# isaac-chandler/cuda-raytracer

Measured on AMD Instinct MI355X. Metric: Mrays/s (live ray segments/s, teapot), higher is better.
Workload: dtype f32

## Files before the change

### cuda-raytracer_amd/csrc/rt_render.hip

```cpp
#include "rt_common.h"

#include <algorithm>
#include <chrono>
#include <cstdio>
#include <cstdlib>
#include <cstring>
#include <string>
#include <thread>
#include <vector>

#include <rccl/rccl.h>

#pragma clang fp contract(off)

int rtamd_render_multi(const rt_scene *scene, const rt_opts *opts, float *fb_out, rt_stats *stats);

using namespace rtamd;

namespace {

#ifndef RT_INFLIGHT
#define RT_INFLIGHT 20
#endif
#ifndef RT_TRACE_OCC
// ... 26 lines not shown
inline int tile_stride(int64_t n_max) {
    return (int)std::max<int64_t>(kTileTarget, (n_max + kSortTile - 1) / kSortTile);
}
constexpr int kBuckets = 65;
constexpr int kInflight = RT_INFLIGHT;
constexpr int kStaggerUs = 4000;
constexpr int kStaggerGroup = 4;
constexpr int kStaggerMinPasses = 8;
constexpr int kStaggerShortUs = 2000;
constexpr int kTraceOccPct = RT_TRACE_OCC;
constexpr uint32_t kDead = 64;
constexpr uint32_t kAccFlag = 0x80000000u;
constexpr int kSpanSlots = 8;
constexpr int kSpanWords = 2 * kSpanSlots;
#ifdef RT_PROFILE
__device__ unsigned long long g_prof[2][14];
#define PROF(i, v) (prof[i] += (v))
#else
#define PROF(i, v) ((void)0)
#endif

struct FastDiv {
    uint32_t m = 0;
    int l = 0;
    static FastDiv of(uint32_t d) {
        FastDiv f;
        if (d > 1) {
            f.l = 32 - __builtin_clz(d - 1);
            f.m = (uint32_t)((((uint64_t)1 << (31 + f.l)) + d - 1) / d);
        }
        return f;
    }
    __device__ __forceinline__ uint32_t div(uint32_t n) const { return l == 0 ? n : (__umulhi(n, m) >> (l - 1)); }
};

struct SlotMap {
    FastDiv by_stripe;
    uint32_t skip, base;
    static SlotMap identity() { return SlotMap{FastDiv::of(0x7fffffffu), 0u, 0u}; }
    static SlotMap of(uint32_t stripe, int count, int index) {
        return SlotMap{FastDiv::of(stripe), (uint32_t)(count - 1) * stripe, (uint32_t)index * stripe};
    }
    __device__ __forceinline__ uint32_t ray(uint32_t s) const { return s + by_stripe.div(s) * skip + base; }
};

template <int FIRST>
__device__ __forceinline__ uint32_t first_ray(const SlotMap &m, uint32_t slot) {
    return FIRST == 2 ? m.ray(slot) : slot;
}

struct PassArgs {
    int rtc;
    uint32_t gen_seed_term;
    FastDiv by_rtc, by_width;
    SlotMap map;
};

__device__ __forceinline__ V3 primary_dir(const DevScene &S, int i, const PassArgs &pa) {
    Rng rng = pcg_seed((uint32_t)i * 0x85810BEAu + pa.gen_seed_term);
    uint32_t z;
    asm volatile("v_mov_b32 %0, 0" : "=v"(z));
    rng.inc += z;
    const uint32_t pixel = pa.by_rtc.div((uint32_t)i);
    const uint32_t yy = pa.by_width.div(pixel);
    const int x = (int)(pixel - yy * (uint32_t)S.width), y = (int)yy;
    const float xc = (x + random01(rng)) * S.inv_w;
    const float yc = (y + random01(rng)) * S.inv_h;
    return normalise(S.tl + xc * S.sr - yc * S.su);
}

#ifndef RT_FUSED_MAX_TRIS
#define RT_FUSED_MAX_TRIS 4096
#endif
#ifndef RT_SORT_GRID
#define RT_SORT_GRID 0
#endif

template <bool SORTED, bool COUNT, int FIRST, bool VSLOT = false>
__global__ __launch_bounds__(kBlock) RT_TRACE_ATTR void trace_kernel(DevScene S, PassArgs pa, const float4 *__restrict__ geo,
                                                       const uint32_t *__restrict__ live_count,
                                                       uint32_t *__restrict__ queue, float2 *__restrict__ hits,
                                                       uint32_t *__restrict__ overflow, Counters *__restrict__ ctr,
                                                       unsigned long long *__restrict__ tspan,
                                                       const uint8_t *__restrict__ slot_bkt = nullptr) {
    __shared__ uint2 stack[(kStackLds + 1) * kBlock];
    const unsigned long long t_start = wall_clock64();
    uint2 *col = stack + threadIdx.x;
    const uint32_t lanes = gridDim.x * kBlock, gl = blockIdx.x * kBlock + threadIdx.x;
    const uint32_t dist_half = lanes * (kStackMax - kStackLds);
    const uint32_t L = __builtin_amdgcn_readfirstlane(*live_count);
    const uint32_t waves = gridDim.x * (kBlock / 64);
    const uint32_t chunk = min((uint32_t)kChunkMax, max((uint32_t)kChunkMin, (L / (4 * waves) + 63) & ~63u));
    uint32_t shard = blockIdx.x % kQueues, tried = 0;
    uint32_t q_next = 0, q_end = 0;
    bool exhausted = false;
    int slot = -1;
    V3 o{0, 0, 0}, d{0, 0, 0};
    float ix = 0, iy = 0, iz = 0, closest = 0;
    bool finite_inv = true;
    bool wave_nonfinite = false;
    int index = -1, sp = 0;
    uint32_t ref = 0;
    int ti = 0, te = 0;
    unsigned pn = 0, iv = 0, tt = 0, nlive = 0;
#ifdef RT_PROFILE
    unsigned long long prof[14] = {0, 0, 0, 0, 0, 0, 0, 0, 0, 0, 0, 0, 0, 0};
#endif
    auto node_step = [&](float4 a, float4 b, float4 c, uint2 kids) -> bool {
        if (COUNT) iv++;
        float t0, t1;
        bool h0, h1;
        slab_pair(a, b, c, o, ix, iy, iz, closest, h0, h1, t0, t1);
        if (__builtin_expect(wave_nonfinite, 0)) {
            float u0, u1;
            const bool g0 = slab(a.x, a.z, b.x, b.z, c.x, c.z, o, ix, iy, iz, closest, u0);
            const bool g1 = slab(a.y, a.w, b.y, b.w, c.y, c.w, o, ix, iy, iz, closest, u1);
            if (!finite_inv) { h0 = g0; h1 = g1; t0 = u0; t1 = u1; }
        }
        const bool both = h0 && h1, any = h0 || h1;
        const bool sel1 = h1 && (!h0 || t0 < t1);
        const uint32_t next_ref = sel1 ? kids.y : kids.x, near_ref = sel1 ? kids.x : kids.y;
        const float next_t = sel1 ? t1 : t0, near_t = sel1 ? t0 : t1;
        col[min(sp, kStackLds) * kBlock] = make_uint2(near_ref, __float_as_uint(near_t));
        if (__builtin_expect(both && sp >= kStackLds, 0)) {
            overflow[(sp - kStackLds) * lanes + gl] = near_ref;
            overflow[dist_half + (sp - kStackLds) * lanes + gl] = __float_as_uint(near_t);
        }
        if (both) sp++;
        ref = any ? next_ref : ref;
        const bool descend = any && !(next_t >= closest);
        bool need = !descend;
        if (descend) {
            if (COUNT) pn++;
            if (ref & kLeaf) {
                leaf_range(S, ref, ti, te);
                need = ti == te;
            }
        }
        return need;
    };
    auto pop_loop = [&](bool need) {
        while (need) {
            PROF(10, 1);
            const bool empty = sp == 0;
            sp = empty ? 0 : sp - 1;
            uint2 e = col[min(sp, kStackLds) * kBlock];
            asm volatile("" : "+v"(e.x), "+v"(e.y));
            if (__builtin_expect(__ballot(sp >= kStackLds) != 0, 0)) {
                if (sp >= kStackLds) {
                    e.x = overflow[(sp - kStackLds) * lanes + gl];
                    e.y = overflow[dist_half + (sp - kStackLds) * lanes + gl];
                }
            }
            const bool take = !empty && !(__uint_as_float(e.y) >= closest);
            slot = empty ? -2 - slot : slot;
            ref = take ? e.x : ref;
            if (COUNT) pn += take ? 1u : 0u;
            const bool leaf = take && (ref & kLeaf);
            if (__builtin_expect(leaf && (ref & kBigLeaf), 0)) {
                leaf_range(S, ref, ti, te);
            } else {
                ti = leaf ? (int)(ref & 0xFFFFFFu) : ti;
                te = leaf ? ti + (int)((ref >> 24) & 0x3Fu) : te;
            }
            need = !empty && (!take || (leaf && ti == te));
        }
    };
    const bool root_internal = !(S.root_ref & kLeaf);
    float4 ra{0, 0, 0, 0}, rb{0, 0, 0, 0}, rc{0, 0, 0, 0};
    uint2 rk{0, 0};
    if (root_internal) {
        const float4 *rr = S.nodes + (size_t)S.root_ref * 4;
        const float4 x0 = rr[0], x1 = rr[1], x2 = rr[2];
        const uint2 k = *reinterpret_cast<const uint2 *>(rr + 3);
#define RT_U(v) __int_as_float(__builtin_amdgcn_readfirstlane(__float_as_int(v)))
        ra = make_float4(RT_U(x0.x), RT_U(x0.y), RT_U(x0.z), RT_U(x0.w));
        rb = make_float4(RT_U(x1.x), RT_U(x1.y), RT_U(x1.z), RT_U(x1.w));
        rc = make_float4(RT_U(x2.x), RT_U(x2.y), RT_U(x2.z), RT_U(x2.w));
#undef RT_U
        rk = make_uint2(__builtin_amdgcn_readfirstlane(k.x), __builtin_amdgcn_readfirstlane(k.y));
    }
    while (true) {
        unsigned long long idle = __ballot(slot < 0);
        if (!exhausted && __popcll(idle) >= (FIRST ? kRefillFirst : kRefill)) {
            PROF(6, 1);
            if (slot <= -2) {
                hits[-2 - slot] = make_float2(closest, __int_as_float(index));
                slot = -1;
            }
            bool fresh = false;
            do {
                bool got = false;
                while (idle && !exhausted) {
                    if (q_next >= q_end) {
                        const uint32_t seg_lo = (uint32_t)(((uint64_t)L * shard) / kQueues);
                        const uint32_t seg_hi = (uint32_t)(((uint64_t)L * (shard + 1)) / kQueues);
                        uint32_t c = 0;
                        if (lane_id() == 0) c = atomicAdd(queue + shard * kQueueStride, chunk);
                        c = __builtin_amdgcn_readfirstlane(__shfl(c, 0)) + seg_lo;
                        if (c >= seg_hi) {
                            shard = (shard + 1) % kQueues;
                            if (++tried == kQueues) exhausted = true;
                            continue;
                        }
                        q_next = c;
                        q_end = min(c + chunk, seg_hi);
                    }
                    const uint32_t avail = q_end - q_next;
                    const uint32_t r = rank_below(idle);
                    const bool take = slot < 0 && r < avail;
                    const unsigned long long took = __ballot(take);
                    if (take) { slot = (int)(q_next + r); fresh = true; got = true; }
                    q_next += (uint32_t)__popcll(took);
                    idle &= ~took;
                }
                if (VSLOT) {
                    if (got && slot_bkt[slot] == kDead) { slot = -1; fresh = false; }
                    idle = __ballot(slot < 0);
                }
            } while (VSLOT && idle && !exhausted);
            if (fresh) {
                {
                    nlive++;
                    if (FIRST) {
                        o = S.cam;
                        d = primary_dir(S, (int)first_ray<FIRST>(pa.map, (uint32_t)slot), pa);
                    } else if (VSLOT) {
                        const float2 *rp = reinterpret_cast<const float2 *>(geo) + (size_t)slot * 3;
                        const float2 r0 = rp[0], r1 = rp[1], r2 = rp[2];
                        o = v3(r0.x, r0.y, r1.x);
                        d = v3(r1.y, r2.x, r2.y);
                    } else {
                        const float4 *rp = geo + (size_t)slot * 2;
                        const float4 r0 = rp[0];
                        const float2 r1 = *reinterpret_cast<const float2 *>(rp + 1);
                        o = v3(r0.x, r0.y, r0.z);
                        d = v3(r0.w, r1.x, r1.y);
                    }
                    ix = 1 / d.x; iy = 1 / d.y; iz = 1 / d.z;
                    finite_inv = __builtin_isfinite(ix) && __builtin_isfinite(iy) && __builtin_isfinite(iz);

                    closest = 1e30f;
                    index = -1;
                    for (int i = 0; i < S.sphere_count; i++) {
                        const float4 sph = S.spheres[i];
                        float t;
                        if (ray_sphere(o, d, v3(sph.x, sph.y, sph.z), sph.w, closest, t)) { closest = t; index = i; }
                    }
                    ref = S.root_ref;
                    sp = 0;
                    if (COUNT) pn++;
                    ti = te = 0;
                    if (ref & kLeaf) {
                        leaf_range(S, ref, ti, te);
                        if (ti == te) {
                            hits[slot] = make_float2(closest, __int_as_float(index));
                            slot = -1;
                        }
                    }
                }
            }
            wave_nonfinite = __ballot(slot >= 0 && !finite_inv) != 0;
            if (root_internal && __ballot(fresh && slot >= 0)) {
                bool need = false;
                if (fresh && slot >= 0) need = node_step(ra, rb, rc, rk);
                pop_loop(need);
            }
        }
        if (!__ballot(slot >= 0)) {
            if (exhausted) break;
            PROF(7, 1);
            continue;
        }
#ifdef RT_PROFILE
        {
            const unsigned long long act = __ballot(slot >= 0), lf = __ballot(slot >= 0 && ti < te);
            PROF(0, 1); PROF(1, __popcll(act)); PROF(2, __popcll(lf));
            PROF(3, lf != 0); PROF(4, (act & ~lf) != 0);
            const bool mixed = lf != 0 && (act & ~lf) != 0;
            PROF(8, mixed);
            if (mixed) PROF(9, min(__popcll(lf), __popcll(act & ~lf)));
            const uintptr_t ra = slot >= 0 ? (uintptr_t)(ti < te ? S.tris + (size_t)ti * 3 : S.nodes + (size_t)ref * 4) : 0;
            const int first = __builtin_ctzll(act);
            const uintptr_t r0 = ((uintptr_t)__shfl((unsigned)(ra >> 32), first) << 32) | __shfl((unsigned)ra, first);
            const unsigned long long same = __ballot(slot >= 0 && ra == r0);
            PROF(12, same == act);
            PROF(13, 4 * __popcll(same) >= 3 * __popcll(act));
        }
#endif
        if (slot < 0) continue;
        bool need = false;
        const bool in_leaf = ti < te;
        const float4 *rec = in_leaf ? S.tris + (size_t)ti * 3 : S.nodes + (size_t)ref * 4;
        const float4 a = rec[0], b = rec[1], c = rec[2];
        uint2 kids = make_uint2(0, 0);
        if (!in_leaf) kids = *reinterpret_cast<const uint2 *>(rec + 3);
        if (in_leaf) {
            const float4 q0 = a, q1 = b;
            const float q2 = c.x;
            if (COUNT) tt++;
            float t;
            const bool hit =
                ray_triangle_flat(o, d, v3(q0.x, q0.y, q0.z), v3(q0.w, q1.x, q1.y), v3(q1.z, q1.w, q2), closest, t);
            closest = hit ? t : closest;
            index = hit ? S.sphere_count + ti : index;
            need = ++ti == te;
        } else {
            need = node_step(a, b, c, kids);
        }
#ifdef RT_PROFILE
        if (__ballot(need)) PROF(5, 1);
#endif
        pop_loop(need);
    }
    if (slot <= -2) hits[-2 - slot] = make_float2(closest, __int_as_float(index));
    Counters *cs = ctr + ((blockIdx.x * (kBlock / 64) + (threadIdx.x >> 6)) & (kCtrSlots - 1));
    const unsigned long long nl = wave_sum(nlive);
    if (COUNT) {
        const unsigned long long a = wave_sum(pn), b = wave_sum(iv), t = wave_sum(tt);
        if (lane_id() == 0) {
            atomicAdd(&cs->pn, a);
            atomicAdd(&cs->iv, b);
            atomicAdd(&cs->tt, t);
            atomicAdd(&cs->st, nl * (unsigned long long)S.sphere_count);
        }
    }
    if (lane_id() == 0 && nl) atomicAdd(&cs->live, nl);
    if (tspan) {
        __syncthreads();
        if (threadIdx.x == 0) {
            atomicMin(&tspan[blockIdx.x % kSpanSlots], t_start);
            atomicMax(&tspan[kSpanSlots + blockIdx.x % kSpanSlots], (unsigned long long)wall_clock64());
        }
    }
#ifdef RT_PROFILE
    prof[11] = wave_sum((unsigned)prof[10]);
    if (lane_id() == 0)
        for (int i = 0; i < 14; i++)
            if (i != 10) atomicAdd(&g_prof[FIRST ? 0 : 1][i], prof[i]);
#endif
}

struct Shaded {
    V3 no, nd, T;
    V3 C;
    uint32_t ray;
    int kind;
    bool acc_holds;
    uint32_t mat;
    bool spec;
};
constexpr uint32_t kSpecBit = 0x80;
struct ShadeIn {
    float2 h;
    uint32_t ray, seed;
    bool acc_holds;
    float4 r0, r1;
    float tz;
};
template <bool SORTED, int FIRST, bool INLINE>
__device__ __forceinline__ ShadeIn shade_in(const PassArgs &pa, int slot, const float4 *__restrict__ geo,
                                            const float *__restrict__ tz, const uint32_t *__restrict__ rid,
                                            const float2 *__restrict__ hits, const uint32_t *__restrict__ seed_of) {
    ShadeIn in{};
    const uint32_t ray0 = first_ray<FIRST>(pa.map, (uint32_t)slot);
    const uint32_t rv = FIRST ? (FIRST == 2 ? ray0 : (uint32_t)slot) : rid[slot];
    in.ray = rv & ~kAccFlag;
    in.acc_holds = (rv & kAccFlag) != 0;
    in.seed = (!FIRST && seed_of) ? seed_of[slot] : (SORTED || FIRST) ? (FIRST == 2 ? ray0 : (uint32_t)slot) : in.ray;
    if (!INLINE) in.h = hits[slot];
    if (!FIRST) {
        in.r0 = geo[(size_t)slot * 2];
        in.r1 = geo[(size_t)slot * 2 + 1];
        in.tz = tz[slot];
    }
    return in;
}
template <bool SORTED, int FIRST, bool INLINE = false, bool SLIM = false>
__device__ __forceinline__ Shaded shade_from(const DevScene &S, const PassArgs &pa, int slot, const ShadeIn &in,
                                             uint32_t seed_term) {
    static_assert(!SLIM || FIRST == 1, "the slim hand-over leaves bounce 0, where T enters as (1,1,1)");
    uint32_t mat = 0;
    bool spec = false;
    Rng rng = pcg_seed(in.seed * 4137874753u + seed_term);
    float closest = in.h.x;
    int index = __float_as_int(in.h.y);
    const uint32_t ray_id = in.ray;
    V3 o, d, T;
    V3 C = v3(0, 0, 0);
    if (FIRST) {
        o = S.cam;
        d = primary_dir(S, (int)(FIRST == 2 ? in.ray : (uint32_t)slot), pa);
        float tx = 1.f, ty = 1.f, tz = 1.f;
        asm volatile("" : "+v"(tx), "+v"(ty), "+v"(tz));
        T = v3(tx, ty, tz);
    } else {
        o = v3(in.r0.x, in.r0.y, in.r0.z);
        d = v3(in.r0.w, in.r1.x, in.r1.y);
        T = v3(in.r1.z, in.r1.w, in.tz);
    }
    if (INLINE) {
        closest = 1e30f;
        index = -1;
        for (int i = 0; i < S.sphere_count; i++) {
            const float4 sph = S.spheres[i];
            float t;
            if (ray_sphere(o, d, v3(sph.x, sph.y, sph.z), sph.w, closest, t)) { closest = t; index = i; }
        }
    }
    V3 no = o, nd = d;
    if (index == -1) {
        C = C + sky_color(S.env, S.env_w, S.env_h, d) * T;
        T = v3(0, 0, 0);
    } else {
        const bool sphere = index < S.sphere_count;
        const uint32_t mi = S.mat_idx[index];
        float4 q = *(sphere ? S.spheres + index : S.tris + (size_t)(index - S.sphere_count) * 3 + 2);
        asm volatile("" : "+v"(q.x), "+v"(q.y), "+v"(q.z), "+v"(q.w));
        no = o + closest * d;
        const V3 normal = sphere ? (1 / q.w) * (no - v3(q.x, q.y, q.z)) : v3(q.y, q.z, q.w);
        const float4 *mp = S.mats + (size_t)mi * 3;
        float4 m0 = mp[0], m1 = mp[1], m2 = mp[2];
        asm volatile("" : "+v"(m0.x), "+v"(m0.y), "+v"(m0.z), "+v"(m0.w), "+v"(m1.x), "+v"(m1.y), "+v"(m1.z),
                          "+v"(m1.w), "+v"(m2.x), "+v"(m2.y), "+v"(m2.z), "+v"(m2.w));
        const Mat m{v3(m0.x, m0.y, m0.z), m0.w, v3(m1.x, m1.y, m1.z), m1.w, v3(m2.x, m2.y, m2.z), m2.w};
        const bool took_spec = scatter(d, normal, m, rng, T, C, nd);
        if (SLIM) {
            spec = took_spec;
            mat = mi;
        }
    }
    return Shaded{no, nd, T, C, ray_id, index == -1 ? 0 : (index < S.sphere_count ? 2 : 1), in.acc_holds, mat, spec};
}
template <bool SORTED, int FIRST, bool INLINE = false, bool SLIM = false>
__device__ __forceinline__ Shaded shade_one(const DevScene &S, const PassArgs &pa, int slot,
                                            const float4 *__restrict__ geo, const float *__restrict__ tz,
                                            const uint32_t *__restrict__ rid, const float2 *__restrict__ hits,
                                            uint32_t seed_term, const uint32_t *__restrict__ seed_of = nullptr) {
    return shade_from<SORTED, FIRST, INLINE, SLIM>(S, pa, slot,
                                                   shade_in<SORTED, FIRST, INLINE>(pa, slot, geo, tz, rid, hits, seed_of),
                                                   seed_term);
}
__device__ __forceinline__ bool has_radiance(V3 c) {
    return ((__float_as_uint(c.x) | __float_as_uint(c.y) | __float_as_uint(c.z)) & 0x7fffffffu) != 0;
}

__device__ __forceinline__ unsigned long long match_bucket(uint32_t b, bool valid);

#ifndef RT_SHADE_WPE
#define RT_SHADE_WPE 8
#endif
#ifndef RT_REPLAY_WPE
#define RT_REPLAY_WPE 8
#endif
#if RT_REPLAY_WPE > 0
#define RT_REPLAY_ATTR __attribute__((amdgpu_waves_per_eu(RT_REPLAY_WPE, RT_REPLAY_WPE)))
#else
#define RT_REPLAY_ATTR
#endif
#if RT_SHADE_WPE > 0
#define RT_SHADE_ATTR __attribute__((amdgpu_waves_per_eu(RT_SHADE_WPE, RT_SHADE_WPE)))
#else
#define RT_SHADE_ATTR
#endif
template <bool SORTED, bool COUNT, int FIRST, bool FUSED, bool INLINE, bool SLIM = false>
__global__ __launch_bounds__(kBlock) RT_SHADE_ATTR void shade_kernel(DevScene S, PassArgs pa, float4 *__restrict__ geo,
                                                       float *__restrict__ tz, uint32_t *__restrict__ rid,
                                                       float4 *__restrict__ acc, uint8_t *__restrict__ bkt,
                                                       const uint32_t *__restrict__ live_count,
                                                       const float2 *__restrict__ hits, uint32_t seed_term, int last,
                                                       Counters *__restrict__ ctr,
                                                       const uint32_t *__restrict__ seed_of = nullptr,
                                                       uint32_t *__restrict__ counts = nullptr, int tiles = 0,
                                                       int home = 0) {
    const int L = (int)__builtin_amdgcn_readfirstlane(*live_count);
    unsigned hit = 0, miss = 0, hit_sphere = 0;
    auto shade_slot = [&](int slot) -> uint32_t {
        const Shaded sh = shade_one<SORTED, FIRST, INLINE, SLIM>(S, pa, slot, geo, tz, rid, hits, seed_term, seed_of);
        const V3 no = sh.no, nd = sh.nd, T = sh.T;
        miss += sh.kind == 0;
        hit += sh.kind != 0;
        hit_sphere += sh.kind == 2;
        const bool dead = is_black(T);
        if (SLIM && !dead && !last) {
            float2 *rec = reinterpret_cast<float2 *>(geo) + (size_t)slot * 3;
            rec[0] = make_float2(no.x, no.y);
            rec[1] = make_float2(no.z, nd.x);
            rec[2] = make_float2(nd.y, nd.z);
            reinterpret_cast<uint16_t *>(tz)[slot] = (uint16_t)sh.mat;
        }
        if (!SLIM && !FUSED && !dead && !last) {
            geo[(size_t)slot * 2] = make_float4(no.x, no.y, no.z, nd.x);
            geo[(size_t)slot * 2 + 1] = make_float4(nd.y, nd.z, T.x, T.y);
            tz[slot] = T.z;
        }
        const bool term = has_radiance(sh.C);
        if (dead || last || (term && !(FIRST && home))) {
            V3 C = sh.C;
            const uint32_t dst = sh.ray;
            if (sh.acc_holds) {
                const float4 a = acc[dst];
                C = v3(a.y, a.z, a.w) + sh.C;
            }
            typedef float f4v __attribute__((ext_vector_type(4)));
            if (dead || last)
                __builtin_nontemporal_store(f4v{T.z, C.x, C.y, C.z}, reinterpret_cast<f4v *>(acc + dst));
            else
                acc[dst] = make_float4(T.z, C.x, C.y, C.z);
        }
        if (!SLIM && !FUSED && !dead && !last && (FIRST || (term && !sh.acc_holds)))
            rid[slot] = sh.ray | (term || sh.acc_holds ? kAccFlag : 0u);
        const uint32_t bk = dead ? kDead : (SORTED ? bucket_of(no, nd, S.min_coord, S.inv_dim) : 0u);
        if (!last) bkt[slot] = (uint8_t)(bk | (SLIM && !dead && sh.spec ? kSpecBit : 0u));
        return bk;
    };
    if (counts && !last) {
        __shared__ uint32_t h[kBuckets];
        const int R = tile_rounds(L), span = kBlock * R;
        for (int tile = blockIdx.x; tile * span < L; tile += gridDim.x) {
            for (int b = threadIdx.x; b < kBuckets; b += kBlock) h[b] = 0;
            __syncthreads();
            const int base = tile * span;
            const int rounds = min(R, (L - base + kBlock - 1) / kBlock);
            for (int r = 0; r < rounds; r++) {
                const int slot = base + r * kBlock + threadIdx.x;
                const bool valid = slot < L;
                const uint32_t bk = valid ? shade_slot(slot) : 0u;
                const unsigned long long peers = match_bucket(bk, valid);
                if (valid && rank_below(peers) == 0) atomicAdd(&h[bk], (uint32_t)__popcll(peers));
            }
            __syncthreads();
            for (int b = threadIdx.x; b < kBuckets; b += kBlock) counts[(size_t)b * tiles + tile] = h[b];
            __syncthreads();
        }
    } else {
        for (int base = blockIdx.x * kBlock; base < L; base += gridDim.x * kBlock) {
            const int slot = base + threadIdx.x;
            if (slot < L) (void)shade_slot(slot);
        }
    }
    if (INLINE) {
        Counters *cs = ctr + ((blockIdx.x * (kBlock / 64) + (threadIdx.x >> 6)) & (kCtrSlots - 1));
        const unsigned long long nl = wave_sum(hit + miss);
        if (lane_id() == 0 && nl) {
            atomicAdd(&cs->live, nl);
            if (COUNT) {
                atomicAdd(&cs->pn, nl);
                atomicAdd(&cs->st, nl * (unsigned long long)S.sphere_count);
            }
        }
    }
    if (COUNT) {
        Counters *cs = ctr + ((blockIdx.x * (kBlock / 64) + (threadIdx.x >> 6)) & (kCtrSlots - 1));
        const unsigned long long h = wave_sum(hit), m = wave_sum(miss), hs = wave_sum(hit_sphere);
        if (lane_id() == 0 && (h | m)) {
            atomicAdd(&cs->hits, h);
            atomicAdd(&cs->misses, m);
            atomicAdd(&cs->hits_sphere, hs);
        }
    }
}

__global__ void fill_live_kernel(uint32_t *__restrict__ live, uint32_t n, int count, uint32_t *__restrict__ queue,
                                 unsigned long long *__restrict__ tspan) {
    const int i = blockIdx.x * blockDim.x + threadIdx.x;
    if (i < count) live[i] = n;
    for (int k = i; k < count * kQueues * kQueueStride; k += blockDim.x) queue[k] = 0;
    if (tspan)
        for (int k = i; k < kSpanWords * count; k += blockDim.x) tspan[k] = (k % kSpanWords) >= kSpanSlots ? 0ull : ~0ull;
}

// ... 269 lines not shown
    if (threadIdx.x == 0) *dst = src ? *src : v;
}

template <bool SORTED, int FIRST, bool INLINE>
__global__ __launch_bounds__(kBlock) RT_REPLAY_ATTR void sort_scatter_shade_kernel(DevScene S, PassArgs pa,
                                                                    const uint8_t *__restrict__ bkt_in,
                                                                    const float4 *__restrict__ geo_in,
                                                                    const float *__restrict__ tz_in,
                                                                    const uint32_t *__restrict__ rid_in,
                                                                    const float2 *__restrict__ hits, uint32_t seed_term,
                                                                    const uint32_t *__restrict__ live_count, int tiles,
                                                                    const uint32_t *__restrict__ offsets,
                                                                    const uint32_t *__restrict__ totals,
                                                                    float4 *__restrict__ geo_out,
                                                                    float *__restrict__ tz_out,
                                                                    uint32_t *__restrict__ rid_out,
                                                                    float4 *__restrict__ acc = nullptr,
                                                                    uint32_t *__restrict__ home_of = nullptr,
                                                                    uint32_t home_base = 0) {
    const bool homes = FIRST == 1 && home_of != nullptr;
    const int n = (int)*live_count;
    __shared__ uint32_t run[kBuckets];
    __shared__ uint32_t wcount[kBlock / 64][kBuckets];
    const int R = tile_rounds(n), span = kBlock * R;
    for (int tile = blockIdx.x; tile * span < n; tile += gridDim.x) {
        bucket_runs(run, offsets, totals, tiles, tile);
        for (int k = threadIdx.x; k < (kBlock / 64) * kBuckets; k += kBlock) (&wcount[0][0])[k] = 0;
        __syncthreads();
        const int wave = threadIdx.x >> 6;
        const int base = tile * span;
        const int rounds = min(R, (n - base + kBlock - 1) / kBlock);
        for (int r = 0; r < rounds; r++) {
            const int item = base + r * kBlock + threadIdx.x;
            const bool valid = item < n;
            const uint32_t b = valid ? bkt_in[item] : 0u;
            const bool move = valid && b != kDead;
            Shaded sh{};
            if (move) sh = shade_one<SORTED, FIRST, INLINE>(S, pa, item, geo_in, tz_in, rid_in, hits, seed_term);
            const unsigned long long peers = match_bucket(b, valid);
            const uint32_t rank = rank_below(peers);
            if (valid && rank == 0) wcount[wave][b] = (uint32_t)__popcll(peers);
            __syncthreads();
            if (move) {
                uint32_t pos = run[b] + rank;
                for (int k = 0; k < wave; k++) pos += wcount[k][b];
                geo_out[(size_t)pos * 2] = make_float4(sh.no.x, sh.no.y, sh.no.z, sh.nd.x);
                geo_out[(size_t)pos * 2 + 1] = make_float4(sh.nd.y, sh.nd.z, sh.T.x, sh.T.y);
                tz_out[pos] = sh.T.z;
                const uint32_t id = homes ? home_base + pos : sh.ray;
                if (homes) {
                    home_of[item] = id;
                    if (has_radiance(sh.C)) acc[id] = make_float4(sh.T.z, sh.C.x, sh.C.y, sh.C.z);
                }
                rid_out[pos] = id | (has_radiance(sh.C) || sh.acc_holds ? kAccFlag : 0u);
            } else if (homes && valid) {
                home_of[item] = (uint32_t)item;
            }
            __syncthreads();
            if (threadIdx.x < kBuckets) {
                uint32_t s = 0;
                for (int k = 0; k < kBlock / 64; k++) { s += wcount[k][threadIdx.x]; wcount[k][threadIdx.x] = 0; }
                run[threadIdx.x] += s;
            }
            __syncthreads();
        }
    }
}


__global__ __launch_bounds__(kBlock) void fill_dead_kernel(uint8_t *__restrict__ bkt, const uint32_t *__restrict__ count) {
    const uint32_t n = *count;
    const uint32_t n16 = n / 16;
    const uint32_t w = kDead * 0x01010101u;
    for (uint32_t i = blockIdx.x * kBlock + threadIdx.x; i < n16; i += gridDim.x * kBlock)
        reinterpret_cast<uint4 *>(bkt)[i] = make_uint4(w, w, w, w);
    for (uint32_t i = n16 * 16 + blockIdx.x * kBlock + threadIdx.x; i < n; i += gridDim.x * kBlock) bkt[i] = (uint8_t)kDead;
}

template <bool COUNT>
__global__ __launch_bounds__(kBlock) RT_SHADE_ATTR void shade_rank_kernel(DevScene S, PassArgs pa,
                                                            const uint8_t *__restrict__ bkt_in,
                                                            const float4 *__restrict__ geo_in,
                                                            const uint16_t *__restrict__ mat_in,
                                                            const float2 *__restrict__ hits, uint32_t seed_term, int last,
                                                            const uint32_t *__restrict__ slot_count, int tiles,
                                                            const uint32_t *__restrict__ offsets,
                                                            const uint32_t *__restrict__ totals,
                                                            float4 *__restrict__ geo_out, float *__restrict__ tz_out,
                                                            uint32_t *__restrict__ rid_out, uint8_t *__restrict__ bkt_out,
                                                            float4 *__restrict__ acc, Counters *__restrict__ ctr) {
    const int n = (int)__builtin_amdgcn_readfirstlane(*slot_count);
    __shared__ uint32_t run[kBuckets];
    __shared__ uint32_t wcount[kBlock / 64][kBuckets];
    unsigned hit = 0, miss = 0, hit_sphere = 0;
    const int R = tile_rounds(n), span = kBlock * R;
    for (int tile = blockIdx.x; tile * span < n; tile += gridDim.x) {
        bucket_runs(run, offsets, totals, tiles, tile);
        for (int k = threadIdx.x; k < (kBlock / 64) * kBuckets; k += kBlock) (&wcount[0][0])[k] = 0;
        __syncthreads();
        const int wave = threadIdx.x >> 6;
        const int base = tile * span;
        const int rounds = min(R, (n - base + kBlock - 1) / kBlock);
        for (int r = 0; r < rounds; r++) {
            const int item = base + r * kBlock + threadIdx.x;
            const bool valid = item < n;
            const uint32_t byte = valid ? bkt_in[item] : 0u;
            const uint32_t b = byte & ~kSpecBit;
            const bool move = valid && b != kDead;
            ShadeIn in{};
            float2 r0{}, r1{}, r2{};
            float4 alb{}, emi{};
            if (move) {
                const float4 *mp = S.mats + (size_t)mat_in[item] * 3;
                in.h = hits[item];
                const float2 *rp = reinterpret_cast<const float2 *>(geo_in) + (size_t)item * 3;
                r0 = rp[0]; r1 = rp[1]; r2 = rp[2];
                alb = mp[byte & kSpecBit ? 1 : 0];
                emi = mp[2];
            }
            const unsigned long long peers = match_bucket(b, valid);
            const uint32_t rank = rank_below(peers);
            if (valid && rank == 0) wcount[wave][b] = (uint32_t)__popcll(peers);
            __syncthreads();
            if (move) {
                uint32_t pos = run[b] + rank;
                for (int k = 0; k < wave; k++) pos += wcount[k][b];
                float one = 1.f;
                asm volatile("" : "+v"(one));
                const V3 ones = v3(one, one, one);
                const V3 T0 = ones * v3(alb.x, alb.y, alb.z);
                in.r0 = make_float4(r0.x, r0.y, r1.x, r1.y);
                in.r1 = make_float4(r2.x, r2.y, T0.x, T0.y);
                in.tz = T0.z;
                in.ray = (uint32_t)item;
                in.acc_holds = has_radiance(v3(0, 0, 0) + v3(emi.x, emi.y, emi.z) * ones);
                in.seed = pos;
                const Shaded sh = shade_from<true, 0>(S, pa, item, in, seed_term);
                const V3 no = sh.no, nd = sh.nd, T = sh.T;
                miss += sh.kind == 0;
                hit += sh.kind != 0;
                hit_sphere += sh.kind == 2;
                const bool dead = is_black(T);
                const bool term = has_radiance(sh.C);
                if (dead || last || term) {
                    V3 C = sh.C;
                    if (sh.acc_holds) {
                        const float4 a = acc[sh.ray];
                        C = v3(a.y, a.z, a.w) + sh.C;
                    }
                    typedef float f4v __attribute__((ext_vector_type(4)));
                    if (dead || last)
                        __builtin_nontemporal_store(f4v{T.z, C.x, C.y, C.z}, reinterpret_cast<f4v *>(acc + sh.ray));
                    else
                        acc[sh.ray] = make_float4(T.z, C.x, C.y, C.z);
                }
                if (!dead && !last) {
                    geo_out[(size_t)pos * 2] = make_float4(no.x, no.y, no.z, nd.x);
                    geo_out[(size_t)pos * 2 + 1] = make_float4(nd.y, nd.z, T.x, T.y);
                    tz_out[pos] = T.z;
                    rid_out[pos] = sh.ray | (term || sh.acc_holds ? kAccFlag : 0u);
                    bkt_out[pos] = (uint8_t)bucket_of(no, nd, S.min_coord, S.inv_dim);
                }
            }
            __syncthreads();
            if (threadIdx.x < kBuckets) {
                uint32_t s = 0;
                for (int k = 0; k < kBlock / 64; k++) { s += wcount[k][threadIdx.x]; wcount[k][threadIdx.x] = 0; }
                run[threadIdx.x] += s;
            }
            __syncthreads();
        }
    }
    if (COUNT) {
        Counters *cs = ctr + ((blockIdx.x * (kBlock / 64) + (threadIdx.x >> 6)) & (kCtrSlots - 1));
        const unsigned long long h = wave_sum(hit), m = wave_sum(miss), hs = wave_sum(hit_sphere);
        if (lane_id() == 0 && (h | m)) {
            atomicAdd(&cs->hits, h);
            atomicAdd(&cs->misses, m);
            atomicAdd(&cs->hits_sphere, hs);
        }
    }
}

constexpr int kAccPixels = 64;
template <bool TILED>
__global__ __launch_bounds__(kBlock) void accumulate_kernel(const float4 *__restrict__ tc, int rtc, int pixels,
                                                            float *__restrict__ sums, SlotMap pix,
                                                            const uint32_t *__restrict__ home_of = nullptr) {
    __shared__ float col[kAccPixels * 20 * 3];
    const int p0 = blockIdx.x * kAccPixels;
    const int np = min(kAccPixels, pixels - p0);
    const int n = np * rtc;
    const float4 *src = tc + (size_t)p0 * rtc;
    for (int e = threadIdx.x; e < n; e += kBlock) {
        const float4 c = TILED     ? tc[(size_t)pix.ray((uint32_t)(p0 + e / rtc)) * rtc + e % rtc]
                         : home_of ? tc[home_of[(size_t)p0 * rtc + e]]
                                   : src[e];
        col[e * 3] = c.y;
        col[e * 3 + 1] = c.z;
        col[e * 3 + 2] = c.w;
    }
    __syncthreads();
    const int t = threadIdx.x;
    if (t >= np) return;
    float sx = 0, sy = 0, sz = 0;
    const float *r = col + t * rtc * 3;
    for (int s = 0; s < rtc; s++) {
        sx = sx + r[s * 3];
        sy = sy + r[s * 3 + 1];
        sz = sz + r[s * 3 + 2];
    }
    const size_t p = TILED ? (size_t)pix.ray((uint32_t)(p0 + t)) : (size_t)(p0 + t);
    sums[p * 3] = sx;
    sums[p * 3 + 1] = sy;
    sums[p * 3 + 2] = sz;
}

__global__ __launch_bounds__(kBlock) void high_pass_kernel(const float *__restrict__ img, float *__restrict__ out,
                                                           float threshold, int pixels) {
    const int i = blockIdx.x * kBlock + threadIdx.x;
// ... 308 lines not shown
    }

    int enqueue_pass(PassCtx &c, int p, float *sums, int64_t &sorted, unsigned long long *tspan) {
        const int before = spp - 20 * p;
        const int rtc = std::min(before, 20);
        const int remaining = before - rtc;
        const int64_t pixels = (int64_t)width * height;
        const int64_t tpix = tile_pixels();
        const int n = (int)(rtc * tpix);
        const int grid = blocks_for(n);
        const int tiles = tile_stride(n);
        const int tgrid = std::min(grid, trace_blocks);
        const int sgrid = std::min(grid, scene.cus * RT_SHADE_BPC);
        const int sort_grid = std::max(1, std::min(max_tiles(n), RT_SORT_GRID > 0 ? RT_SORT_GRID : scene.cus * 8));
        hipStream_t st = c.stream;
        int cur = 0;
        if (n == 0) {
            for (int k = 0; pass_events && k < 3 * bounces + 2 * (bounces - 1); k++) {
                hipEvent_t e = c.event();
                if (!e) return rtamd::fail(RT_E_HIP, "hipEventCreate failed");
                HIPCHK(hipEventRecord(e, st));
            }
            HIPCHK(hipMemsetAsync(sums, 0, (size_t)pixels * 3 * sizeof(float), st));
            return RT_OK;
        }
        hipLaunchKernelGGL(fill_live_kernel, dim3(1), dim3(256), 0, st, c.live.p, (uint32_t)n, bounces + 1, c.queue.p, tspan);
        const uint32_t stripe_px = (uint32_t)(tile_rows * width);
        const SlotMap pix = tiled() ? SlotMap::of(stripe_px, tile_count, tile_index) : SlotMap::identity();
        const SlotMap map = tiled() ? SlotMap::of(stripe_px * (uint32_t)rtc, tile_count, tile_index) : SlotMap::identity();
        const PassArgs pa{rtc, 709579u * (uint32_t)remaining, FastDiv::of((uint32_t)rtc), FastDiv::of((uint32_t)width),
                          map};
        for (int b = 0; b < bounces; b++) {
            const uint32_t seed_term = 279220567u * (uint32_t)(remaining * 20 + b);
            hipEvent_t e0 = nullptr, em = nullptr, e1 = nullptr;
            if (pass_events) {
                e0 = c.event(); em = c.event(); e1 = c.event();
                if (!e0 || !em || !e1) return rtamd::fail(RT_E_HIP, "hipEventCreate failed");
                HIPCHK(hipEventRecord(e0, st));
            }
            const uint32_t *lv = c.live.p + b;
            uint32_t *q = c.queue.p + (size_t)b * kQueues * kQueueStride;
            const bool last = b + 1 == bounces;
            const bool v0 = vre && b == 0, v1 = vre && b == 1;
            const bool fuse_b = !v0 && !v1 && (fused || b <= fused_upto);
            uint32_t *hist = (shade_hist || v0) && !last && !v1 ? c.sort_counts.p : nullptr;
#define RT_PROCESS3(SORTED, COUNT, FIRST)                                                                        \
    do {                                                                                                         \
        if (!inline_hits)                                                                                        \
            hipLaunchKernelGGL((trace_kernel<SORTED, COUNT, FIRST>), dim3(tgrid), dim3(kBlock), 0, st, scene.ds, pa, \
                               c.geo[cur].p, lv, q, c.hits.p, c.overflow.p, scene.ctr.p,                         \
                               tspan ? tspan + kSpanWords * b : nullptr);                                        \
        if (em) HIPCHK(hipEventRecord(em, st));                                                                  \
        if (inline_hits)                                                                                         \
            hipLaunchKernelGGL((shade_kernel<SORTED, COUNT, FIRST, true, true>), dim3(sgrid), dim3(kBlock), 0, st,\
                               scene.ds, pa, c.geo[cur].p, c.tz[cur].p, c.rid[cur].p, c.acc.p, c.bkt.p, lv, c.hits.p, \
                               seed_term, (int)last, scene.ctr.p, nullptr, hist, tiles, (int)(home && b == 0));  \
        else if (fuse_b)                                                                                         \
            hipLaunchKernelGGL((shade_kernel<SORTED, COUNT, FIRST, true, false>), dim3(sgrid), dim3(kBlock), 0, \
                               st, scene.ds, pa, c.geo[cur].p, c.tz[cur].p, c.rid[cur].p, c.acc.p, c.bkt.p, lv, c.hits.p, \
                               seed_term, (int)last, scene.ctr.p, nullptr, hist, tiles, (int)(home && b == 0));  \
        else                                                                                                     \
            hipLaunchKernelGGL((shade_kernel<SORTED, COUNT, FIRST, false, false>), dim3(sgrid), dim3(kBlock), 0, \
                               st, scene.ds, pa, c.geo[cur].p, c.tz[cur].p, c.rid[cur].p, c.acc.p, c.bkt.p, lv, c.hits.p, \
                               seed_term, (int)last, scene.ctr.p, nullptr, hist, tiles, (int)(home && b == 0));  \
    } while (0)
#define RT_PROCESS(SORTED, COUNT)                                                                                \
    do {                                                                                                         \
        if (b == 0) RT_PROCESS3(SORTED, COUNT, 1); else RT_PROCESS3(SORTED, COUNT, 0);                           \
    } while (0)
            if (v0) {
#define RT_V0PROCESS(COUNT)                                                                                      \
    do {                                                                                                         \
        hipLaunchKernelGGL((trace_kernel<true, COUNT, 1>), dim3(tgrid), dim3(kBlock), 0, st, scene.ds, pa,       \
                           c.geo[cur].p, lv, q, c.hits.p, c.overflow.p, scene.ctr.p,                             \
                           tspan ? tspan + kSpanWords * b : nullptr);                                            \
        if (em) HIPCHK(hipEventRecord(em, st));                                                                  \
        hipLaunchKernelGGL((shade_kernel<true, COUNT, 1, false, false, true>), dim3(sgrid), dim3(kBlock), 0, st, \
                           scene.ds, pa, c.geo[cur].p, c.tz[cur].p, c.rid[cur].p, c.acc.p, c.bkt.p, lv, c.hits.p, \
                           seed_term, (int)last, scene.ctr.p, nullptr, hist, tiles, 0);                          \
    } while (0)
                if (counters) RT_V0PROCESS(true); else RT_V0PROCESS(false);
#undef RT_V0PROCESS
            } else if (v1) {
#define RT_VPROCESS(COUNT)                                                                                       \
    do {                                                                                                         \
        hipLaunchKernelGGL((trace_kernel<true, COUNT, 0, true>), dim3(tgrid), dim3(kBlock), 0, st, scene.ds, pa, \
                           c.geo[cur].p, c.live.p, q, c.hits.p, c.overflow.p, scene.ctr.p,                       \
                           tspan ? tspan + kSpanWords * b : nullptr, c.bkt.p);                                   \
        if (em) HIPCHK(hipEventRecord(em, st));                                                                  \
        hipLaunchKernelGGL((shade_rank_kernel<COUNT>), dim3(sort_grid), dim3(kBlock), 0, st, scene.ds, pa, c.bkt.p, \
                           c.geo[cur].p, reinterpret_cast<const uint16_t *>(c.tz[cur].p), c.hits.p, seed_term,   \
                           (int)last, c.live.p, tiles, c.sort_offsets.p, c.sort_totals.p, c.geo[1 - cur].p,      \
                           c.tz[1 - cur].p, c.rid[1 - cur].p, c.bkt1.p, c.acc.p, scene.ctr.p);                   \
    } while (0)
                if (counters) RT_VPROCESS(true); else RT_VPROCESS(false);
#undef RT_VPROCESS
                cur = 1 - cur;
            } else if (sort) {
                if (counters) RT_PROCESS(true, true); else RT_PROCESS(true, false);
            } else {
                if (b == 0 && tiled()) {
                    if (counters) RT_PROCESS3(false, true, 2); else RT_PROCESS3(false, false, 2);
                } else if (counters) RT_PROCESS(false, true); else RT_PROCESS(false, false);
            }
#undef RT_PROCESS
#undef RT_PROCESS3
            HIPCHK(hipGetLastError());
            if (pass_events) HIPCHK(hipEventRecord(e1, st));
            if (b + 1 != bounces) {
                hipEvent_t s0 = nullptr, s1 = nullptr;
                if (pass_events) {
                    s0 = c.event(); s1 = c.event();
                    if (!s0 || !s1) return rtamd::fail(RT_E_HIP, "hipEventCreate failed");
                    HIPCHK(hipEventRecord(s0, st));
                }
                const uint8_t *bk = v1 ? c.bkt1.p : c.bkt.p;
                if (!hist)
                    hipLaunchKernelGGL(sort_hist_kernel, dim3(sort_grid), dim3(kBlock), 0, st, bk, lv, tiles,
                                       c.sort_counts.p);
                hipLaunchKernelGGL(sort_scan_kernel, dim3(kBuckets), dim3(kBlock), 0, st, c.sort_counts.p, lv, tiles,
                                   c.sort_offsets.p, c.sort_totals.p, c.live.p + b + 1);
                if (v0) {
                    if (b + 2 != bounces)
                        hipLaunchKernelGGL(fill_dead_kernel, dim3(sort_grid), dim3(kBlock), 0, st, c.bkt1.p, c.live.p + 1);
                } else if (fuse_b) {
#define RT_FSC2(SO, FI, IN)                                                                                      \
    hipLaunchKernelGGL((sort_scatter_shade_kernel<SO, FI, IN>), dim3(sort_grid), dim3(kBlock), 0, st, scene.ds, pa, \
                       c.bkt.p, c.geo[cur].p, c.tz[cur].p, c.rid[cur].p, c.hits.p, seed_term, lv, tiles,          \
                       c.sort_offsets.p, c.sort_totals.p, c.geo[1 - cur].p, c.tz[1 - cur].p, c.rid[1 - cur].p,    \
                       c.acc.p, home && b == 0 ? c.home_of.p : nullptr, home_base)
#define RT_FSC(SO, FI) do { if (inline_hits) RT_FSC2(SO, FI, true); else RT_FSC2(SO, FI, false); } while (0)
                    if (sort) {
                        if (b == 0) RT_FSC(true, 1); else RT_FSC(true, 0);
                    } else {
                        if (b == 0 && tiled()) RT_FSC(false, 2); else if (b == 0) RT_FSC(false, 1); else RT_FSC(false, 0);
                    }
#undef RT_FSC
#undef RT_FSC2
                } else if (b == 0 && tiled())
                    hipLaunchKernelGGL(sort_scatter_kernel<2>, dim3(sort_grid), dim3(kBlock), 0, st, c.bkt.p, c.geo[cur].p,
                                       c.tz[cur].p, c.rid[cur].p, lv, tiles, c.sort_offsets.p, c.sort_totals.p,
                                       c.geo[1 - cur].p, c.tz[1 - cur].p, c.rid[1 - cur].p, pa.map);
                else if (b == 0)
                    hipLaunchKernelGGL(sort_scatter_kernel<1>, dim3(sort_grid), dim3(kBlock), 0, st, c.bkt.p, c.geo[cur].p,
                                       c.tz[cur].p, c.rid[cur].p, lv, tiles, c.sort_offsets.p, c.sort_totals.p,
                                       c.geo[1 - cur].p, c.tz[1 - cur].p, c.rid[1 - cur].p, pa.map);
                else
                    hipLaunchKernelGGL(sort_scatter_kernel<0>, dim3(sort_grid), dim3(kBlock), 0, st, bk, c.geo[cur].p,
                                       c.tz[cur].p, c.rid[cur].p, lv, tiles, c.sort_offsets.p, c.sort_totals.p,
                                       c.geo[1 - cur].p, c.tz[1 - cur].p, c.rid[1 - cur].p, pa.map);
                HIPCHK(hipGetLastError());
                if (pass_events) HIPCHK(hipEventRecord(s1, st));
                if (!v0) cur = 1 - cur;
                if (sort) sorted += n;
            }
        }
        if (bounces == 0) {
            HIPCHK(hipMemsetAsync(sums, 0, (size_t)pixels * 3 * sizeof(float), st));
        } else if (!tiled()) {
            hipLaunchKernelGGL(accumulate_kernel<false>, dim3((unsigned)((pixels + kAccPixels - 1) / kAccPixels)),
                               dim3(kBlock), 0, st, c.acc.p, rtc, (int)pixels, sums, pix, home ? c.home_of.p : nullptr);
        } else {
            HIPCHK(hipMemsetAsync(sums, 0, (size_t)pixels * 3 * sizeof(float), st));
            if (tpix > 0)
                hipLaunchKernelGGL(accumulate_kernel<true>, dim3((unsigned)((tpix + kAccPixels - 1) / kAccPixels)),
                                   dim3(kBlock), 0, st, c.acc.p, rtc, (int)tpix, sums, pix);
        }
        HIPCHK(hipGetLastError());
        return RT_OK;
    }

    int wait_event(hipEvent_t e) {
        if (!xpoll) {
            HIPCHK(hipEventSynchronize(e));
// ... 776 lines not shown
```

Before: 14700.

## Slim bounce-1 hand-over record to direction plus hit distance, recompute origin

The bounce-0 shade now stores a single float4 per slot (direction and hit distance t) instead of a 24-byte origin/direction record. The bounce-1 trace kernel rebuilds the origin from the camera, the primary direction and t. It writes only the hit index plus the hit point into a separate buffer, so the shade-rank kernel no longer reloads and recomputes it. This cuts memory traffic between stages, at the cost of recomputing primary directions in trace. The rebuilt origin may differ slightly in floating point, and the hit-point buffer placed after geo is a possible aliasing risk.

```diff
diff --git a/cuda-raytracer_amd/csrc/rt_render.hip b/cuda-raytracer_amd/csrc/rt_render.hip
--- a/cuda-raytracer_amd/csrc/rt_render.hip
+++ b/cuda-raytracer_amd/csrc/rt_render.hip
@@ -132,12 +132,19 @@
                                                        uint32_t *__restrict__ queue, float2 *__restrict__ hits,
                                                        uint32_t *__restrict__ overflow, Counters *__restrict__ ctr,
                                                        unsigned long long *__restrict__ tspan,
-                                                       const uint8_t *__restrict__ slot_bkt = nullptr) {
+                                                       const uint8_t *__restrict__ slot_bkt = nullptr,
+                                                       float *__restrict__ hit_org = nullptr) {
     __shared__ uint2 stack[(kStackLds + 1) * kBlock];
     const unsigned long long t_start = wall_clock64();
     uint2 *col = stack + threadIdx.x;
     const uint32_t lanes = gridDim.x * kBlock, gl = blockIdx.x * kBlock + threadIdx.x;
     const uint32_t dist_half = lanes * (kStackMax - kStackLds);
+    auto overflow_lane = [&]() -> uint32_t {
+        if (!VSLOT) return gl;
+        uint32_t t = threadIdx.x;
+        asm volatile("" : "+v"(t));
+        return blockIdx.x * kBlock + t;
+    };
     const uint32_t L = __builtin_amdgcn_readfirstlane(*live_count);
     const uint32_t waves = gridDim.x * (kBlock / 64);
     const uint32_t chunk = min((uint32_t)kChunkMax, max((uint32_t)kChunkMin, (L / (4 * waves) + 63) & ~63u));
@@ -173,8 +180,8 @@
         const float next_t = sel1 ? t1 : t0, near_t = sel1 ? t0 : t1;
         col[min(sp, kStackLds) * kBlock] = make_uint2(near_ref, __float_as_uint(near_t));
         if (__builtin_expect(both && sp >= kStackLds, 0)) {
-            overflow[(sp - kStackLds) * lanes + gl] = near_ref;
-            overflow[dist_half + (sp - kStackLds) * lanes + gl] = __float_as_uint(near_t);
+            overflow[(sp - kStackLds) * lanes + overflow_lane()] = near_ref;
+            overflow[dist_half + (sp - kStackLds) * lanes + overflow_lane()] = __float_as_uint(near_t);
         }
         if (both) sp++;
         ref = any ? next_ref : ref;
@@ -198,8 +205,8 @@
             asm volatile("" : "+v"(e.x), "+v"(e.y));
             if (__builtin_expect(__ballot(sp >= kStackLds) != 0, 0)) {
                 if (sp >= kStackLds) {
-                    e.x = overflow[(sp - kStackLds) * lanes + gl];
-                    e.y = overflow[dist_half + (sp - kStackLds) * lanes + gl];
+                    e.x = overflow[(sp - kStackLds) * lanes + overflow_lane()];
+                    e.y = overflow[dist_half + (sp - kStackLds) * lanes + overflow_lane()];
                 }
             }
             const bool take = !empty && !(__uint_as_float(e.y) >= closest);
@@ -214,6 +221,18 @@
                 te = leaf ? ti + (int)((ref >> 24) & 0x3Fu) : te;
             }
             need = !empty && (!take || (leaf && ti == te));
+        }
+    };
+    auto store_result = [&](int s) {
+        if (VSLOT) {
+            reinterpret_cast<int *>(hits)[s] = index;
+            if (index != -1) {
+                const V3 no = o + closest * d;
+                float *p = hit_org + (size_t)s * 3;
+                p[0] = no.x; p[1] = no.y; p[2] = no.z;
+            }
+        } else {
+            hits[s] = make_float2(closest, __int_as_float(index));
         }
     };
     const bool root_internal = !(S.root_ref & kLeaf);
@@ -235,7 +254,7 @@
         if (!exhausted && __popcll(idle) >= (FIRST ? kRefillFirst : kRefill)) {
             PROF(6, 1);
             if (slot <= -2) {
-                hits[-2 - slot] = make_float2(closest, __int_as_float(index));
+                store_result(-2 - slot);
                 slot = -1;
             }
             bool fresh = false;
@@ -276,10 +295,9 @@
                         o = S.cam;
                         d = primary_dir(S, (int)first_ray<FIRST>(pa.map, (uint32_t)slot), pa);
                     } else if (VSLOT) {
-                        const float2 *rp = reinterpret_cast<const float2 *>(geo) + (size_t)slot * 3;
-                        const float2 r0 = rp[0], r1 = rp[1], r2 = rp[2];
-                        o = v3(r0.x, r0.y, r1.x);
-                        d = v3(r1.y, r2.x, r2.y);
+                        const float4 r = geo[slot];
+                        o = S.cam + r.w * primary_dir(S, slot, pa);
+                        d = v3(r.x, r.y, r.z);
                     } else {
                         const float4 *rp = geo + (size_t)slot * 2;
                         const float4 r0 = rp[0];
@@ -304,7 +322,7 @@
                     if (ref & kLeaf) {
                         leaf_range(S, ref, ti, te);
                         if (ti == te) {
-                            hits[slot] = make_float2(closest, __int_as_float(index));
+                            store_result(slot);
                             slot = -1;
                         }
                     }
@@ -363,7 +381,7 @@
 #endif
         pop_loop(need);
     }
-    if (slot <= -2) hits[-2 - slot] = make_float2(closest, __int_as_float(index));
+    if (slot <= -2) store_result(-2 - slot);
     Counters *cs = ctr + ((blockIdx.x * (kBlock / 64) + (threadIdx.x >> 6)) & (kCtrSlots - 1));
     const unsigned long long nl = wave_sum(nlive);
     if (COUNT) {
@@ -399,6 +417,7 @@
     bool acc_holds;
     uint32_t mat;
     bool spec;
+    float t;
 };
 constexpr uint32_t kSpecBit = 0x80;
 struct ShadeIn {
@@ -407,6 +426,7 @@
     bool acc_holds;
     float4 r0, r1;
     float tz;
+    const float *org;
 };
 template <bool SORTED, int FIRST, bool INLINE>
 __device__ __forceinline__ ShadeIn shade_in(const PassArgs &pa, int slot, const float4 *__restrict__ geo,
@@ -426,10 +446,11 @@
     }
     return in;
 }
-template <bool SORTED, int FIRST, bool INLINE = false, bool SLIM = false>
+template <bool SORTED, int FIRST, bool INLINE = false, bool SLIM = false, bool LEAN = false>
 __device__ __forceinline__ Shaded shade_from(const DevScene &S, const PassArgs &pa, int slot, const ShadeIn &in,
                                              uint32_t seed_term) {
     static_assert(!SLIM || FIRST == 1, "the slim hand-over leaves bounce 0, where T enters as (1,1,1)");
+    static_assert(!LEAN || (!FIRST && !INLINE), "the lean result is the bounce-1 trace kernel's");
     uint32_t mat = 0;
     bool spec = false;
     Rng rng = pcg_seed(in.seed * 4137874753u + seed_term);
@@ -466,8 +487,9 @@
         const bool sphere = index < S.sphere_count;
         const uint32_t mi = S.mat_idx[index];
         float4 q = *(sphere ? S.spheres + index : S.tris + (size_t)(index - S.sphere_count) * 3 + 2);
+        if (LEAN) no = v3(in.org[0], in.org[1], in.org[2]);
         asm volatile("" : "+v"(q.x), "+v"(q.y), "+v"(q.z), "+v"(q.w));
-        no = o + closest * d;
+        if (!LEAN) no = o + closest * d;
         const V3 normal = sphere ? (1 / q.w) * (no - v3(q.x, q.y, q.z)) : v3(q.y, q.z, q.w);
         const float4 *mp = S.mats + (size_t)mi * 3;
         float4 m0 = mp[0], m1 = mp[1], m2 = mp[2];
@@ -480,7 +502,8 @@
             mat = mi;
         }
     }
-    return Shaded{no, nd, T, C, ray_id, index == -1 ? 0 : (index < S.sphere_count ? 2 : 1), in.acc_holds, mat, spec};
+    return Shaded{no, nd, T, C, ray_id, index == -1 ? 0 : (index < S.sphere_count ? 2 : 1), in.acc_holds, mat, spec,
+                  closest};
 }
 template <bool SORTED, int FIRST, bool INLINE = false, bool SLIM = false>
 __device__ __forceinline__ Shaded shade_one(const DevScene &S, const PassArgs &pa, int slot,
@@ -533,10 +556,7 @@
         hit_sphere += sh.kind == 2;
         const bool dead = is_black(T);
         if (SLIM && !dead && !last) {
-            float2 *rec = reinterpret_cast<float2 *>(geo) + (size_t)slot * 3;
-            rec[0] = make_float2(no.x, no.y);
-            rec[1] = make_float2(no.z, nd.x);
-            rec[2] = make_float2(nd.y, nd.z);
+            geo[slot] = make_float4(nd.x, nd.y, nd.z, sh.t);
             reinterpret_cast<uint16_t *>(tz)[slot] = (uint16_t)sh.mat;
         }
         if (!SLIM && !FUSED && !dead && !last) {
@@ -972,7 +992,8 @@
                                                             const uint8_t *__restrict__ bkt_in,
                                                             const float4 *__restrict__ geo_in,
                                                             const uint16_t *__restrict__ mat_in,
-                                                            const float2 *__restrict__ hits, uint32_t seed_term, int last,
+                                                            const int *__restrict__ hit_idx,
+                                                            const float *__restrict__ hit_org, uint32_t seed_term, int last,
                                                             const uint32_t *__restrict__ slot_count, int tiles,
                                                             const uint32_t *__restrict__ offsets,
                                                             const uint32_t *__restrict__ totals,
@@ -998,13 +1019,12 @@
             const uint32_t b = byte & ~kSpecBit;
             const bool move = valid && b != kDead;
             ShadeIn in{};
-            float2 r0{}, r1{}, r2{};
+            float4 rec{};
             float4 alb{}, emi{};
             if (move) {
                 const float4 *mp = S.mats + (size_t)mat_in[item] * 3;
-                in.h = hits[item];
-                const float2 *rp = reinterpret_cast<const float2 *>(geo_in) + (size_t)item * 3;
-                r0 = rp[0]; r1 = rp[1]; r2 = rp[2];
+                in.h = make_float2(0.f, __int_as_float(hit_idx[item]));
+                rec = geo_in[item];
                 alb = mp[byte & kSpecBit ? 1 : 0];
                 emi = mp[2];
             }
@@ -1019,13 +1039,14 @@
                 asm volatile("" : "+v"(one));
                 const V3 ones = v3(one, one, one);
                 const V3 T0 = ones * v3(alb.x, alb.y, alb.z);
-                in.r0 = make_float4(r0.x, r0.y, r1.x, r1.y);
-                in.r1 = make_float4(r2.x, r2.y, T0.x, T0.y);
+                in.r0 = make_float4(0.f, 0.f, 0.f, rec.x);
+                in.r1 = make_float4(rec.y, rec.z, T0.x, T0.y);
                 in.tz = T0.z;
+                in.org = hit_org + (size_t)item * 3;
                 in.ray = (uint32_t)item;
                 in.acc_holds = has_radiance(v3(0, 0, 0) + v3(emi.x, emi.y, emi.z) * ones);
                 in.seed = pos;
-                const Shaded sh = shade_from<true, 0>(S, pa, item, in, seed_term);
+                const Shaded sh = shade_from<true, 0, false, false, true>(S, pa, item, in, seed_term);
                 const V3 no = sh.no, nd = sh.nd, T = sh.T;
                 miss += sh.kind == 0;
                 hit += sh.kind != 0;
@@ -1500,14 +1521,16 @@
                 if (counters) RT_V0PROCESS(true); else RT_V0PROCESS(false);
 #undef RT_V0PROCESS
             } else if (v1) {
+                float *hit_org = reinterpret_cast<float *>(c.geo[cur].p + n);
 #define RT_VPROCESS(COUNT)                                                                                       \
     do {                                                                                                         \
         hipLaunchKernelGGL((trace_kernel<true, COUNT, 0, true>), dim3(tgrid), dim3(kBlock), 0, st, scene.ds, pa, \
                            c.geo[cur].p, c.live.p, q, c.hits.p, c.overflow.p, scene.ctr.p,                       \
-                           tspan ? tspan + kSpanWords * b : nullptr, c.bkt.p);                                   \
+                           tspan ? tspan + kSpanWords * b : nullptr, c.bkt.p, hit_org);                          \
         if (em) HIPCHK(hipEventRecord(em, st));                                                                  \
         hipLaunchKernelGGL((shade_rank_kernel<COUNT>), dim3(sort_grid), dim3(kBlock), 0, st, scene.ds, pa, c.bkt.p, \
-                           c.geo[cur].p, reinterpret_cast<const uint16_t *>(c.tz[cur].p), c.hits.p, seed_term,   \
+                           c.geo[cur].p, reinterpret_cast<const uint16_t *>(c.tz[cur].p),                        \
+                           reinterpret_cast<const int *>(c.hits.p), hit_org, seed_term,                          \
                            (int)last, c.live.p, tiles, c.sort_offsets.p, c.sort_totals.p, c.geo[1 - cur].p,      \
                            c.tz[1 - cur].p, c.rid[1 - cur].p, c.bkt1.p, c.acc.p, scene.ctr.p);                   \
     } while (0)
```

Result: faster. 14930, median of 6 (+1.6%).
